# Xinjie-Q/Boosting-NeRV

Hardware: AMD Instinct MI355X
Metric: train frames/sec (higher is better)
Workload: dtype fp32; 1 GPU; NeRV-boost 1.5M (1489577 params, fc_dim 30) train step on a synthetic Bunny-shaped clip 132x3x720x1280: decoder fwd + Fusion10_freq + bwd + fused Adan; frames resident in HBM; global_batch=1, per_gpu_batch=1, parallelism=dp1, hipgraph=True, rccl_ranks=0, collective_in_graph=False

## Files before the change

boosting_nerv_amd/csrc/conv.hip:

```cpp
#include "common.h"
#include "sidejob.h"
#include "conv_common.h"

int bnerv_convbf_try(hipStream_t st, const bnerv_conv_desc& d, int vec, int ksplit, int chunks_per_split);
namespace bnerv_conv { struct KArgs; }
int bnerv_conv4_try(hipStream_t st, bnerv_conv::KArgs& ka);
int bnerv_convs_try(hipStream_t st, const bnerv_conv_desc& d, int vec, int ksplit);
int bnerv_head3_try(hipStream_t st, const bnerv_conv_desc& d);
bool bnerv_convs_shape_ok(const bnerv_conv_desc& d, int vec);
int bnerv_stem_dgrad_try(hipStream_t st, const bnerv_conv_desc& d);
size_t bnerv_stem_dgrad_ws_bytes(const bnerv_conv_desc& d);
int bnerv_convs_tiles(int H, int W);

namespace {
using namespace bnerv_conv;

#ifndef BNERV_ABL
#define BNERV_ABL 0
#endif
constexpr bool ABL_NO_MFMA = BNERV_ABL == 1 || BNERV_ABL == 3 || BNERV_ABL == 4;
constexpr bool ABL_NO_LOAD = BNERV_ABL == 2 || BNERV_ABL == 4;
constexpr bool ABL_NO_STORE = BNERV_ABL == 2 || BNERV_ABL == 3;
struct Item { int g, b, ty0, tx0, tile, ks; };

__device__ __forceinline__ Item decode_item(const KArgs& ka, int it) {
    const int tiles = ka.tiles_x * ka.tiles_y;
    Item r;
    r.ks = 0;
    if (ka.ksplit > 1) { r.ks = it % ka.ksplit; it /= ka.ksplit; }
    r.tile = it % tiles;
    const int rest = it / tiles;
    r.b = rest % ka.d.B;
    r.g = rest / ka.d.B;
    r.ty0 = (r.tile / ka.tiles_x) * TH;
    r.tx0 = (r.tile % ka.tiles_x) * TW;
    return r;
}

template <int IN>
__device__ __forceinline__ float load_in_scalar(const bnerv_conv_desc& d, int b, int ci, int gy, int gx) {
    if constexpr (IN == BNERV_IN_UNSHUFFLE) {
        const int s = d.in_s, s2 = s * s;
        const int c = ci / s2, rem = ci - c * s2, i = rem / s, j = rem - i * s;
        return d.x[(((size_t)b * (d.Cin / s2) + c) * (size_t)(d.H * s) + (size_t)(gy * s + i)) * (size_t)(d.W * s) + (size_t)(gx * s + j)];
    } else {
        const size_t idx = (((size_t)b * d.Cin + ci) * d.H + gy) * (size_t)d.W + gx;
        float sc = 1.f, sh = 0.f, aux = 0.f;
        if constexpr (IN == BNERV_IN_AFFINE || IN == BNERV_IN_GELU_AFFINE) { sc = 1.0f + d.scale[b * d.Cin + ci]; sh = d.shift[b * d.Cin + ci]; }
        if constexpr (IN == BNERV_IN_TANHGRAD) aux = d.aux0[idx];
        return xform1<IN>(d.x[idx], sc, sh, aux);
    }
}

template <int KS, int IN>
__device__ __forceinline__ void stage_scalar(const bnerv_conv_desc& d, float* s_in, int b, int c0, int nch, int ty0, int tx0) {
    using G = Geo<KS>;
    const int n_el = nch * G::PLANE_RAW;
    for (int i0 = threadIdx.x; i0 < n_el; i0 += 256 * 8) {
        float v[8];
// ... 1549 lines not shown
    else BNERV_REQUIRE(d.Cout == d.wCo && d.Cin == d.wCi, "conv_igemm: weight dims mismatch");
    if (d.in_mode == BNERV_IN_AFFINE || d.in_mode == BNERV_IN_GELU_AFFINE) BNERV_REQUIRE(d.scale && d.shift, "conv_igemm: affine prologue needs scale/shift");
    if (d.in_mode == BNERV_IN_TANHGRAD) BNERV_REQUIRE(d.aux0, "conv_igemm: tanh-grad prologue needs aux0");
    if (d.ep_mode == BNERV_EP_BIAS_RES) BNERV_REQUIRE(d.aux0, "conv_igemm: residual epilogue needs aux0");
    if (d.ep_mode == BNERV_EP_DGELU) BNERV_REQUIRE(d.aux0 && d.scale && d.partial && d.out_s == 1, "conv_igemm: DGELU epilogue args");
    if (d.ep_mode == BNERV_EP_DSIN) BNERV_REQUIRE(d.aux0 && d.aux1 && d.scale && d.partial && d.out_s == 1, "conv_igemm: DSIN epilogue args");
    if (d.ep_mode == BNERV_EP_DGELU_SAVED) BNERV_REQUIRE(d.aux0 && d.aux1 && d.scale && d.partial && d.out_s == 1, "conv_igemm: DGELU_SAVED epilogue args");
    if (d.ep_mode == BNERV_EP_BIAS_GELU) BNERV_REQUIRE(d.out_s == 1, "conv_igemm: BIAS_GELU epilogue needs a stride-1 output");
    if (d.in_mode == BNERV_IN_UNSHUFFLE && d.in_s == 1) d.in_mode = BNERV_IN_PLAIN;
    ka.tiles_x = cdiv(d.W, TW);
    ka.tiles_y = cdiv(d.H, TH);
    ka.vec = conv_vec_ok(d);
    hipStream_t st = reinterpret_cast<hipStream_t>(stream);
    ka.ksplit = 1;
    ka.chunks_per_split = 0;
    ka.magic_tiles = ka.magic_tiles_x = 0;
    if (d.ep_mode == BNERV_EP_PLAIN && d.partial != nullptr) {
        const SplitPlan p = plan_split(d);
        ka.ksplit = p.ksplit;
        ka.chunks_per_split = p.chunks_per_split;
    }
    {
        const char* hf = getenv("BNERV_HEAD_FWD");
        if (!(hf && hf[0] == '0') && d.k == 1 && d.in_mode == BNERV_IN_PLAIN && d.ep_mode == BNERV_EP_BIAS_TANH && d.out_s == 1 && ka.vec && !d.transposed &&
            d.Cin == 12 && d.Cout == 3 && d.wCo == 3 && d.wCi == 12 && ((size_t)d.H * d.W) % 4 == 0 && d.B <= 65535) {
            const int hw4 = (int)(((size_t)d.H * d.W) / 4);
            hipLaunchKernelGGL((head1x1_fwd_kernel<3, 12>), dim3(cdiv(hw4, 256), d.B), dim3(256), 0, st, d, hw4);
            BNERV_LAUNCH_CHECK("head1x1_fwd");
            return BNERV_OK;
        }
    }
    if (d.k == 1 && d.in_mode == BNERV_IN_TANHGRAD && d.ep_mode == BNERV_EP_PLAIN && d.out_s == 1 && ka.vec && ka.ksplit == 1 &&
        d.Cin <= HEAD_KMAX && d.Cout <= HEAD_CMAX && ((size_t)d.H * d.W) % 4 == 0 && d.B <= 65535) {
        const int hw4 = (int)(((size_t)d.H * d.W) / 4);
        hipLaunchKernelGGL(head1x1_dgrad_kernel, dim3(cdiv(hw4, 256), d.B), dim3(256), 0, st, d, hw4);
        BNERV_LAUNCH_CHECK("head1x1_dgrad");
        return BNERV_OK;
    }
    if (d.k == 3 && (d.Cout == 3 || d.Cin == 3) && ka.ksplit == 1) {
        const int rh = bnerv_head3_try(st, d);
        if (rh != 1) return rh;
    }
    if (d.ep_mode == BNERV_EP_PLAIN && d.partial != nullptr) {
        const int rs = bnerv_stem_dgrad_try(st, d);
        if (rs != 1) return rs;
    }
    {
        const int rs = bnerv_convs_try(st, d, ka.vec, ka.ksplit);
        if (rs != 1) return rs;
    }
    int rc = bnerv_convbf_try(st, d, ka.vec, ka.ksplit, ka.chunks_per_split);
    if (rc == 1) {
        ka.magic_tiles = ka.magic_tiles_x = 0;
        rc = bnerv_conv4_try(st, ka);
        if (rc == 1) rc = d.k == 1 ? launch_mode<1>(st, ka) : launch_mode<3>(st, ka);
    }
    if (rc != BNERV_OK || ka.ksplit == 1) return rc;
    return bnerv_reduce_slabs(stream, d.partial, ka.ksplit, d.B * d.Cout * d.H * d.W, d.out);
}
```

boosting_nerv_amd/csrc/conv4.hip:

```cpp
#include "conv4_body.h"

namespace {
using namespace bnerv_conv;
using namespace bnerv_q4;

template <int IN, int EP>
__global__ __launch_bounds__(256, 3) void conv_q4_kernel(const KArgs ka, const SidePack side) {
    conv_q4_body<IN, EP>(ka, side, (int)blockIdx.x, (int)gridDim.x);
}

template <int IN, int EP>
int launch_q4(hipStream_t st, KArgs& ka) {
    q4_prepare(ka);
    const size_t lds = q4_lds_bytes();
    static int blocks_per_cu = 0;
    if (blocks_per_cu == 0) {
        int nb = 0;
        if (hipOccupancyMaxActiveBlocksPerMultiprocessor(&nb, reinterpret_cast<const void*>(&conv_q4_kernel<IN, EP>), 256, lds) != hipSuccess || nb < 1) nb = 1;
        blocks_per_cu = nb;
    }
    int grid = 256 * blocks_per_cu;
    if (grid > ka.total_items) grid = ka.total_items;
    SidePack side;
    bnerv_side_take(ka.d.ctx, &side, 2 * grid);
    hipLaunchKernelGGL((conv_q4_kernel<IN, EP>), dim3(grid), dim3(256), lds, st, ka, side);
    BNERV_LAUNCH_CHECK("conv_q4");
    return BNERV_OK;
}

}

#ifdef BNERV_TRACE
extern "C" int bnerv_debug_trace4_read(void* host) { return (int)hipMemcpyFromSymbol(host, HIP_SYMBOL(g_trace4), sizeof(g_trace4)); }
#endif
int bnerv_conv4_try(hipStream_t st, bnerv_conv::KArgs& ka) {
    const bnerv_conv_desc& d = ka.d;
    static const bool off = [] { const char* e = getenv("BNERV_Q4"); return e && e[0] == '0'; }();
    if (off) return 1;
    if (!q4_shape_ok(ka)) return 1;
    const int in = d.in_mode, ep = d.ep_mode;
#define BNERV_CASE(I, E) if (in == I && ep == E) return launch_q4<I, E>(st, ka);
    BNERV_CASE(BNERV_IN_PLAIN, BNERV_EP_BIAS)
    BNERV_CASE(BNERV_IN_PLAIN, BNERV_EP_BIAS_SIN)
    BNERV_CASE(BNERV_IN_PLAIN, BNERV_EP_PLAIN)
    BNERV_CASE(BNERV_IN_PLAIN, BNERV_EP_DGELU_SAVED)
    BNERV_CASE(BNERV_IN_PLAIN, BNERV_EP_DSIN)
#undef BNERV_CASE
    return 1;
}
```

boosting_nerv_amd/csrc/conv4_body.h:

```cpp
#pragma once
#include "common.h"
#include "sidejob.h"
#include "conv_common.h"

namespace bnerv_q4 {
using bnerv_conv::TH; using bnerv_conv::TW; using bnerv_conv::Geo; using bnerv_conv::KArgs; using bnerv_conv::LItem; using bnerv_conv::OOB;
using bnerv_conv::i32x4; using bnerv_conv::make_rsrc; using bnerv_conv::bload; using bnerv_conv::bstore; using bnerv_conv::fast_div;
using bnerv_conv::div_magic; using bnerv_conv::xform1; using bnerv_conv::LEAN_MAX_BYTES;


#ifndef BNERV_ABL4
#define BNERV_ABL4 0
#endif
constexpr int Q4_NCH = 12;
constexpr int Q4_NG = 3;
constexpr int Q4_NQD = 9 * Q4_NG;
constexpr int Q4_NWR = (Q4_NQD + 3) / 4;
constexpr int Q4_QPAD = Q4_NWR * 4;

#ifdef BNERV_TRACE
__device__ unsigned long long g_trace4[1024 * 4 * 6 * 8];
#define TRACE(slot) do { if (lane == 0 && vb < 1024 && trace_iter < 6) g_trace4[((vb * 4 + wave) * 6 + trace_iter) * 8 + (slot)] = __builtin_amdgcn_s_memtime(); } while (0)
#else
#define TRACE(slot) do {} while (0)
#endif

template <int G>
__device__ __forceinline__ f32x4 mfma_q(float a, float w, f32x4 c) {
    return __builtin_amdgcn_mfma_f32_4x4x1f32(a, w, c, 0, 0, 4 + G);
}
__device__ __forceinline__ f32x4 mfma_qsel(int g, float a, float w, f32x4 c) {
    switch (g) {
        case 0: return mfma_q<0>(a, w, c);
        case 1: return mfma_q<1>(a, w, c);
        case 2: return mfma_q<2>(a, w, c);
        default: return mfma_q<3>(a, w, c);
    }
}

__device__ __forceinline__ void dma16(i32x4 rsrc, unsigned voff, unsigned soff, unsigned lds_addr) {
    asm volatile("s_mov_b32 m0, %3\n\tbuffer_load_dwordx4 %0, %1, %2 offen lds" ::"v"(voff), "s"(rsrc), "s"(soff), "s"(lds_addr) : "memory", "m0");
}
template <int N>
__device__ __forceinline__ void q4_wait_dma() {
    asm volatile("s_waitcnt vmcnt(%0)" ::"n"(N) : "memory");
}

template <int IN, int EP>
__device__ __forceinline__ void conv_q4_body(const KArgs& ka, const SidePack& side, const int vb, const int vgrid) {
    using G = Geo<3>;
    constexpr int NSLOT = Q4_NCH * G::ROWS * G::SEGS;
    constexpr int NPRE = (NSLOT + 255) / 256;
    constexpr int S_IN = NPRE * 256 * 4;
    constexpr int S_W = Q4_NCH * Q4_QPAD * 4;
    constexpr bool AFF = (IN == BNERV_IN_AFFINE);
    constexpr bool RED = (EP == BNERV_EP_DSIN || EP == BNERV_EP_DGELU_SAVED);
    constexpr bool TWO_OUT = (EP == BNERV_EP_BIAS_SIN || EP == BNERV_EP_BIAS_GELU);
    static_assert(IN == BNERV_IN_PLAIN || IN == BNERV_IN_AFFINE, "prologues of the 12-channel layers");
    static_assert(G::PLANE == G::PLANE_RAW && S_IN >= Q4_NCH * G::PLANE, "slot offset = 16 * slot index");
    const bnerv_conv_desc& d = ka.d;
    extern __shared__ __attribute__((aligned(16))) float smem[];
    float* s_in = smem;
    float* s_w = smem + 2 * S_IN;
    float* s_red = s_w + S_W;
    float* s_aff = s_red + 256;
    float* s_beta = s_aff + 32;

    const int tid = threadIdx.x, lane = tid & 63;
    const int wave = __builtin_amdgcn_readfirstlane(tid >> 6);
    const int lj = lane & 3, lb = lane >> 2;
    const int Cin = d.Cin, Cout = d.Cout, H = d.H, W = d.W;
    const int tiles_x = ka.tiles_x, tiles_y = ka.tiles_y;
    { const int trace_iter = 5; (void)trace_iter; TRACE(0); }

    const int xcd = vb & 7, lbk = vb >> 3;
    const int nlb = (vgrid - xcd + 7) >> 3;
    const int per = ka.total_items >> 3, extra = ka.total_items & 7;
    const int r0 = xcd * per + min(xcd, extra), r1 = r0 + per + (xcd < extra ? 1 : 0);
    int itx = r0 + lbk;
    if (itx >= r1) { side_run_hosted(side, smem, vb, vgrid); return; }
    const int step_q = fast_div(nlb, ka.magic_tiles_x), step_r = nlb - step_q * tiles_x;
    LItem it;
    {
        const int tiles = tiles_x * tiles_y;
        it.b = fast_div(itx, ka.magic_tiles);
        const int t = itx - it.b * tiles;
        it.ty = fast_div(t, ka.magic_tiles_x);
        it.tx = t - it.ty * tiles_x;
    }
    auto advance = [&](LItem a) {
        a.tx += step_r;
        a.ty += step_q;
        if (a.tx >= tiles_x) { a.tx -= tiles_x; ++a.ty; }
        while (a.ty >= tiles_y) { a.ty -= tiles_y; ++a.b; }
        return a;
    };

    auto slot_geom = [&](int k, int& c, int& r, int& sg) {
        const int sidx = tid + k * 256;
        c = sidx / (G::ROWS * G::SEGS);
        const int rem = sidx - c * (G::ROWS * G::SEGS);
        r = rem / G::SEGS;
        sg = rem - r * G::SEGS;
    };
    auto slot_inside = [&](int k, int ty0, int tx0) {
        int c, r, sg;
        slot_geom(k, c, r, sg);
        const int gy = ty0 + r - G::PAD, gx = tx0 + 4 * sg - G::XOFF;
        return (unsigned)gy < (unsigned)H && (unsigned)gx < (unsigned)W;
    };
    unsigned voff[NPRE];
#pragma unroll
    for (int k = 0; k < NPRE; ++k) {
        int c, r, sg;
        slot_geom(k, c, r, sg);
        voff[k] = (tid + k * 256 < NSLOT && c < Cin) ? (unsigned)(((c * H + r) * W + 4 * sg) * 4) : OOB;
    }
    const unsigned shift = (unsigned)((G::PAD * W + G::XOFF) * 4);
    const unsigned in_bytes = (unsigned)((size_t)d.B * Cin * H * W * 4) + shift;
    const unsigned out_bytes = (unsigned)((size_t)d.B * Cout * H * W * 4);
    i32x4 rx;
    {
        const uintptr_t base = reinterpret_cast<uintptr_t>(d.x) - shift;
        rx[0] = (int)(unsigned)(base & 0xffffffffu);
        rx[1] = (int)(unsigned)((base >> 32) & 0xffffu);
        rx[2] = (int)in_bytes;
        rx[3] = 0x00020000;
    }
    const __amdgpu_buffer_rsrc_t ro = make_rsrc(d.out, 0, out_bytes);
    const __amdgpu_buffer_rsrc_t ro2 = make_rsrc((TWO_OUT && d.out2) ? d.out2 : d.out, 0, out_bytes);
    const __amdgpu_buffer_rsrc_t ra0 = make_rsrc(d.aux0 ? d.aux0 : d.out, 0, out_bytes);
    const __amdgpu_buffer_rsrc_t ra1 = make_rsrc(d.aux1 ? d.aux1 : d.out, 0, out_bytes);
    const __amdgpu_buffer_rsrc_t ra2 = make_rsrc(d.aux2 ? d.aux2 : d.out, 0, out_bytes);
    const unsigned lds_in = (unsigned)(uintptr_t)(__attribute__((address_space(3))) float*)s_in + (unsigned)wave * 1024u;

    const unsigned ovoff = (unsigned)(((lj * H + (lb >> 3)) * W + 4 * (lb & 7)) * 4);
    const unsigned nstep = (unsigned)(4 * H * W * 4);
    float bias_l[Q4_NG];
#pragma unroll
    for (int n = 0; n < Q4_NG; ++n) bias_l[n] = (EP != BNERV_EP_PLAIN && !RED && d.bias && 4 * n + lj < Cout) ? d.bias[4 * n + lj] : 0.f;
    float scl[Q4_NG];
#pragma unroll
    for (int n = 0; n < Q4_NG; ++n) scl[n] = 0.f;

    auto issue = [&](const LItem& a, int buf) {
        const int ty0 = a.ty * TH, tx0 = a.tx * TW;
        const unsigned sb = (unsigned)((((a.b * Cin) * H + ty0) * W + tx0) * 4);
        const unsigned lbase = lds_in + (unsigned)buf * (unsigned)(S_IN * 4);
        const bool interior = ty0 >= G::PAD && ty0 + TH + G::PAD <= H && tx0 >= G::XOFF && tx0 + TW + G::XOFF <= W;
        if (interior) {
#pragma unroll
            for (int k = 0; k < NPRE; ++k) dma16(rx, (BNERV_ABL4 == 2 && d.B > 0) ? OOB : voff[k], sb, lbase + (unsigned)k * 4096u);
        } else {
#pragma unroll
            for (int k = 0; k < NPRE; ++k) dma16(rx, slot_inside(k, ty0, tx0) ? voff[k] : OOB, sb, lbase + (unsigned)k * 4096u);
        }
    };
    auto flush_partials = [&](const LItem& a, const int set) {
        if (wave == 0 && lane < 32) {
            const int q = lane >> 4, c = lane & 15;
            const float* sr = s_red + set * 128;
            const float s = ((sr[(0 * 2 + q) * 16 + c] + sr[(1 * 2 + q) * 16 + c]) + sr[(2 * 2 + q) * 16 + c]) + sr[(3 * 2 + q) * 16 + c];
            const size_t row = (size_t)(a.ty * tiles_x + a.tx) * d.B + a.b;
            if (c < Cout) d.partial[(row * 2 + q) * Cout + c] = s;
        }
    };

    float wr[Q4_NCH][Q4_NWR];
    float beta_l[Q4_NG];
#pragma unroll
    for (int n = 0; n < Q4_NG; ++n) beta_l[n] = 0.f;
    auto fetch_affine = [&](int b) {
        const int c = tid & 15;
        float v = 0.f;
        if (tid < 32 && c < Cin) v = tid < 16 ? 1.0f + d.scale[b * Cin + c] : d.shift[b * Cin + c];
        return v;
    };
    auto load_weights = [&]() {
#pragma unroll
        for (int ci = 0; ci < Q4_NCH; ++ci) {
            const float f = AFF ? s_aff[ci] : 1.0f;
#pragma unroll
            for (int v = 0; v < Q4_NWR; ++v) {
                const float w = s_w[(ci * Q4_QPAD + 4 * v + (lane >> 4)) * 4 + lj];
                wr[ci][v] = AFF ? w * f : w;
            }
        }
    };
    auto fold_shift = [&]() {
        if constexpr (AFF) {
            if (tid < 9 * 16) {
                const int tap = tid >> 4, co = tid & 15;
                float acc_ = 0.f;
                if (co < 4 * Q4_NG) {
#pragma unroll
                    for (int ci = 0; ci < Q4_NCH; ++ci) acc_ = fmaf(s_aff[16 + ci], s_w[(ci * Q4_QPAD + tap * Q4_NG + (co >> 2)) * 4 + (co & 3)], acc_);
                }
                s_beta[tid] = acc_;
            }
            lds_barrier();
#pragma unroll
            for (int n = 0; n < Q4_NG; ++n) {
                float t = 0.f;
#pragma unroll
                for (int tap = 0; tap < 9; ++tap) t += s_beta[tap * 16 + 4 * n + lj];
                beta_l[n] = t;
            }
        }
    };

    int aff_b = -1, ep_b = -1;
    float aff_v = 0.f;
    { const int trace_iter = 5; (void)trace_iter; TRACE(2); }
    if constexpr (AFF) { aff_v = fetch_affine(it.b); aff_b = it.b; }
    issue(it, 0);
    { const int trace_iter = 5; (void)trace_iter; TRACE(3); }
    {
        constexpr int NWV = (S_W + 255) / 256;
        float wv[NWV];
#pragma unroll
        for (int u = 0; u < NWV; ++u) {
            const int e = tid + u * 256;
            const int j = e & 3, cq = e >> 2;
            const int ci = cq / Q4_QPAD, q = cq - ci * Q4_QPAD;
            const int tap = q / Q4_NG, n = q - tap * Q4_NG;
            const int co = 4 * n + j;
            float v = 0.f;
            if (e < S_W && q < Q4_NQD && co < Cout && ci < Cin)
                v = d.transposed ? d.w[(ci * d.wCi + co) * 9 + (8 - tap)] : d.w[(co * d.wCi + ci) * 9 + tap];
            wv[u] = v;
        }
        { const int trace_iter = 5; (void)trace_iter; TRACE(4); }
        if constexpr (AFF) { if (tid < 32) s_aff[tid] = aff_v; }
#pragma unroll
        for (int u = 0; u < NWV; ++u)
            if (tid + u * 256 < S_W) s_w[tid + u * 256] = wv[u];
    }
    q4_wait_dma<0>();
    lds_barrier();
    { const int trace_iter = 5; (void)trace_iter; TRACE(5); }
    load_weights();
    fold_shift();
    { const int trace_iter = 5; (void)trace_iter; TRACE(6); }
    { const int trace_iter = 5; (void)trace_iter; TRACE(1); }
    const float* a_base = s_in + (2 * wave + (lane >> 5)) * G::RS + (lane & 31) + G::COL0;
    int buf = 0;
    LItem prev = it;
    bool have_prev = false;
    int red_set = 0;
    int trace_iter = 0; (void)trace_iter;
    for (; itx < r1; itx += nlb, ++trace_iter, red_set ^= 1) {
        TRACE(0);
        f32x4 acc[Q4_NG];
#pragma unroll
        for (int n = 0; n < Q4_NG; ++n) acc[n] = f32x4{0.f, 0.f, 0.f, 0.f};
        const bool has_next = itx + nlb < r1;
        LItem nxt = it;
        if (has_next) nxt = advance(it);
        TRACE(1);
        if (has_next) issue(nxt, buf ^ 1);
        TRACE(2);
        if constexpr (RED) { if (have_prev) flush_partials(prev, red_set ^ 1); }
        constexpr int NAUX = (EP == BNERV_EP_BIAS_RES) ? 1 : (EP == BNERV_EP_DGELU_SAVED) ? 2 : (EP == BNERV_EP_DSIN) ? 3 : 0;
        f32x4 ax0[NAUX ? Q4_NG : 1], ax1[NAUX >= 2 ? Q4_NG : 1], ax2[NAUX >= 3 ? Q4_NG : 1];
        unsigned so[Q4_NG], vo[Q4_NG];
        bool ch_ok[Q4_NG];
        {
            const int ty0 = it.ty * TH, tx0 = it.tx * TW;
            const unsigned ob = (unsigned)((((it.b * Cout) * H + ty0 + 2 * wave) * W + tx0) * 4);
            const bool full = ty0 + TH <= H && tx0 + TW <= W;
            bool px_ok = true;
            if (!full) px_ok = (ty0 + 2 * wave + (lb >> 3) < H) && (tx0 + 4 * (lb & 7) < W);
#pragma unroll
            for (int n = 0; n < Q4_NG; ++n) {
                so[n] = ob + (unsigned)n * nstep;
                ch_ok[n] = px_ok && (4 * n + lj < Cout);
                vo[n] = (ch_ok[n] && !(BNERV_ABL4 == 2 && d.B > 0)) ? ovoff : OOB;
            }
            if constexpr (NAUX >= 1) {
#pragma unroll
                for (int n = 0; n < Q4_NG; ++n) ax0[n] = bload(ra0, vo[n], so[n]);
            }
            if constexpr (NAUX >= 2) {
#pragma unroll
                for (int n = 0; n < Q4_NG; ++n) ax1[n] = bload(ra1, vo[n], so[n]);
            }
            if constexpr (NAUX >= 3) {
#pragma unroll
                for (int n = 0; n < Q4_NG; ++n) ax2[n] = d.aux2 ? bload(ra2, vo[n], so[n]) : f32x4{1.f, 1.f, 1.f, 1.f};
            }
        }
        float a_cur[3], a_nxt[3];
        if (BNERV_ABL4 != 1 || d.B < 0) {
#pragma unroll
        for (int kx = 0; kx < 3; ++kx) a_cur[kx] = a_base[kx];
#pragma unroll
        for (int ci = 0; ci < Q4_NCH; ++ci) {
#pragma unroll
            for (int ky = 0; ky < 3; ++ky) {
                const int nci = ky == 2 ? ci + 1 : ci, nky = ky == 2 ? 0 : ky + 1;
                if (nci < Q4_NCH) {
#pragma unroll
                    for (int kx = 0; kx < 3; ++kx) a_nxt[kx] = a_base[nci * G::PLANE + nky * G::RS + kx];
                }
                __builtin_amdgcn_sched_barrier(0);
#pragma unroll
                for (int kx = 0; kx < 3; ++kx)
#pragma unroll
                    for (int n = 0; n < Q4_NG; ++n) {
                        const int q = (ky * 3 + kx) * Q4_NG + n;
                        acc[n] = mfma_qsel(q & 3, a_cur[kx], wr[ci][q >> 2], acc[n]);
                    }
                __builtin_amdgcn_sched_barrier(0);
#pragma unroll
                for (int kx = 0; kx < 3; ++kx) a_cur[kx] = a_nxt[kx];
            }
        }
        }
        TRACE(3);
        TRACE(4);
        TRACE(5);
        {
            const int ty0 = it.ty * TH, tx0 = it.tx * TW;
            if constexpr (RED) {
                if (it.b != ep_b) {
#pragma unroll
                    for (int n = 0; n < Q4_NG; ++n) scl[n] = 4 * n + lj < Cout ? 1.0f + d.scale[it.b * Cout + 4 * n + lj] : 0.f;
                    ep_b = it.b;
                }
            }
            if constexpr (RED) {
#pragma unroll
                for (int n = 0; n < Q4_NG; ++n) { if (!ch_ok[n]) acc[n] = f32x4{0.f, 0.f, 0.f, 0.f}; }
            }
            if constexpr (AFF) {
                const bool border = ty0 == 0 || ty0 + TH >= H || tx0 == 0 || tx0 + TW >= W;
                if (!border) {
#pragma unroll
                    for (int n = 0; n < Q4_NG; ++n) acc[n] += beta_l[n];
                } else {
                    const int gy = ty0 + 2 * wave + (lb >> 3), gx0 = tx0 + 4 * (lb & 7);
#pragma unroll
                    for (int n = 0; n < Q4_NG; ++n) {
                        float col[3];
#pragma unroll
                        for (int kx = 0; kx < 3; ++kx) {
                            float t = 0.f;
#pragma unroll
                            for (int ky = 0; ky < 3; ++ky) t += ((unsigned)(gy + ky - 1) < (unsigned)H) ? s_beta[(ky * 3 + kx) * 16 + 4 * n + lj] : 0.f;
                            col[kx] = t;
                        }
#pragma unroll
                        for (int e = 0; e < 4; ++e) {
                            float t = 0.f;
#pragma unroll
                            for (int kx = 0; kx < 3; ++kx) t += ((unsigned)(gx0 + e + kx - 1) < (unsigned)W) ? col[kx] : 0.f;
                            acc[n][e] += t;
                        }
                    }
                }
            }
            if constexpr (EP == BNERV_EP_BIAS || EP == BNERV_EP_PLAIN) {
#pragma unroll
                for (int n = 0; n < Q4_NG; ++n) bstore(ro, vo[n], so[n], acc[n] + bias_l[n]);
            } else if constexpr (EP == BNERV_EP_BIAS_SIN) {
#pragma unroll
                for (int n = 0; n < Q4_NG; ++n) {
                    f32x4 sv, cv;
                    sincos4_f(acc[n] + bias_l[n], &sv, &cv);
                    bstore(ro, vo[n], so[n], sv);
                    bstore(ro2, d.out2 ? vo[n] : OOB, so[n], cv);
                }
            } else if constexpr (EP == BNERV_EP_BIAS_GELU) {
#pragma unroll
                for (int n = 0; n < Q4_NG; ++n) {
                    f32x4 hv, gv;
                    gelu_pair4_f(acc[n] + bias_l[n], &hv, &gv);
                    bstore(ro, vo[n], so[n], hv);
                    bstore(ro2, d.out2 ? vo[n] : OOB, so[n], gv);
                }
            } else if constexpr (EP == BNERV_EP_BIAS_RES) {
#pragma unroll
                for (int n = 0; n < Q4_NG; ++n) bstore(ro, vo[n], so[n], acc[n] + bias_l[n] + ax0[n]);
            } else {
                float ps[Q4_NG], pt[Q4_NG];
#pragma unroll
                for (int n = 0; n < Q4_NG; ++n) {
                    f32x4 r;
                    const f32x4 v = acc[n];
                    ps[n] = 0.f; pt[n] = 0.f;
                    if constexpr (EP == BNERV_EP_DGELU_SAVED) {
#pragma unroll
                        for (int e = 0; e < 4; ++e) { r[e] = v[e] * scl[n] * ax0[n][e]; ps[n] = fmaf(v[e], ax1[n][e], ps[n]); pt[n] += v[e]; }
                    } else {
#pragma unroll
                        for (int e = 0; e < 4; ++e) { r[e] = (ax1[n][e] + v[e] * scl[n]) * ax2[n][e]; ps[n] = fmaf(v[e], ax0[n][e], ps[n]); pt[n] += v[e]; }
                    }
                    bstore(ro, vo[n], so[n], r);
                }
#pragma unroll
                for (int n = 0; n < Q4_NG; ++n) {
#pragma unroll
                    for (int off = 4; off < 64; off <<= 1) {
                        ps[n] += __shfl_xor(ps[n], off, 64);
                        pt[n] += __shfl_xor(pt[n], off, 64);
                    }
                }
                if (lane < 4) {
#pragma unroll
                    for (int n = 0; n < Q4_NG; ++n) { s_red[red_set * 128 + (wave * 2 + 0) * 16 + 4 * n + lane] = ps[n]; s_red[red_set * 128 + (wave * 2 + 1) * 16 + 4 * n + lane] = pt[n]; }
                }
            }
        }
        TRACE(6);
        if (has_next) {
            q4_wait_dma<(TWO_OUT ? 2 : 1) * Q4_NG>();
            lds_barrier();
            if constexpr (AFF) {
                if (nxt.b != aff_b) {
                    const float v = fetch_affine(nxt.b);
                    if (tid < 32) s_aff[tid] = v;
                    lds_barrier();
                    load_weights();
                    fold_shift();
                    aff_b = nxt.b;
                }
            }
            buf ^= 1;
            a_base = s_in + buf * S_IN + (2 * wave + (lane >> 5)) * G::RS + (lane & 31) + G::COL0;
        }
        TRACE(7);
        prev = it;
        have_prev = true;
        it = nxt;
    }
    if constexpr (RED) {
        lds_barrier();
        flush_partials(prev, red_set ^ 1);
    }
    side_run_hosted(side, smem, vb, vgrid);
}


inline size_t q4_lds_bytes() {
    using G = Geo<3>;
    constexpr int NSLOT = Q4_NCH * G::ROWS * G::SEGS;
    constexpr int NPRE = (NSLOT + 255) / 256;
    return ((size_t)2 * NPRE * 256 * 4 + (size_t)Q4_NCH * Q4_QPAD * 4 + 256 + 32 + 9 * 16) * sizeof(float);
}
inline bool q4_shape_ok(const KArgs& ka) {
    const bnerv_conv_desc& d = ka.d;
    const size_t cmax = (size_t)(d.Cin > d.Cout ? d.Cin : d.Cout);
    return ka.vec && d.k == 3 && d.out_s == 1 && d.Cin > 8 && d.Cin <= Q4_NCH && d.Cout <= 4 * Q4_NG && ka.ksplit == 1 &&
           (size_t)d.B * cmax * d.H * d.W * 4 + (size_t)(d.W + 4) * 4 < LEAN_MAX_BYTES;
}
inline void q4_prepare(KArgs& ka) {
    ka.ngroups = 1;
    ka.total_items = ka.d.B * ka.tiles_x * ka.tiles_y;
    ka.nq_total = 3;
    ka.w_resident = 1;
    ka.magic_tiles = div_magic(ka.tiles_x * ka.tiles_y);
    ka.magic_tiles_x = div_magic(ka.tiles_x);
}

}
```

Before: 687.8 frames/s.

## Add Winograd F(2x2,3x3) forward conv kernel for 12-channel full-resolution layers

Adds a Winograd-domain 3x3 convolution kernel that transforms input tiles and filters, multiplies them with fp32 MFMA, and inverse-transforms the result. It is used by default only for the affine-input, bias+residual forward layer at 720x1280 with at most 12 channels, and is gated by the BNERV_WINO environment variable. The affine shift is folded into a per-output beta term, with border correction at image edges. The goal is to cut MFMA and LDS work for these small-channel, high-resolution convolutions, at the cost of extra transform arithmetic and slight numerical differences.

New measurement: 687.3 frames/s (median of 2 runs). About the same (-0.1%).

```diff
diff --git a/boosting_nerv_amd/csrc/conv.hip b/boosting_nerv_amd/csrc/conv.hip
--- a/boosting_nerv_amd/csrc/conv.hip
+++ b/boosting_nerv_amd/csrc/conv.hip
@@ -5,6 +5,7 @@
 int bnerv_convbf_try(hipStream_t st, const bnerv_conv_desc& d, int vec, int ksplit, int chunks_per_split);
 namespace bnerv_conv { struct KArgs; }
 int bnerv_conv4_try(hipStream_t st, bnerv_conv::KArgs& ka);
+int bnerv_convw_try(hipStream_t st, bnerv_conv::KArgs& ka);
 int bnerv_convs_try(hipStream_t st, const bnerv_conv_desc& d, int vec, int ksplit);
 int bnerv_head3_try(hipStream_t st, const bnerv_conv_desc& d);
 bool bnerv_convs_shape_ok(const bnerv_conv_desc& d, int vec);
@@ -1660,7 +1661,8 @@
     int rc = bnerv_convbf_try(st, d, ka.vec, ka.ksplit, ka.chunks_per_split);
     if (rc == 1) {
         ka.magic_tiles = ka.magic_tiles_x = 0;
-        rc = bnerv_conv4_try(st, ka);
+        rc = bnerv_convw_try(st, ka);
+        if (rc == 1) rc = bnerv_conv4_try(st, ka);
         if (rc == 1) rc = d.k == 1 ? launch_mode<1>(st, ka) : launch_mode<3>(st, ka);
     }
     if (rc != BNERV_OK || ka.ksplit == 1) return rc;
diff --git a/boosting_nerv_amd/csrc/convw.hip b/boosting_nerv_amd/csrc/convw.hip
--- /dev/null
+++ b/boosting_nerv_amd/csrc/convw.hip
@@ -0,0 +1,384 @@
+#include "common.h"
+#include "sidejob.h"
+#include "conv_common.h"
+#include <cstdlib>
+
+namespace {
+using namespace bnerv_conv;
+
+constexpr int WN_NCH = 12;
+constexpr int WN_NQ = 3;
+constexpr int WN_SU = WN_NQ * 4 * 64 * 4;
+
+__device__ __forceinline__ void wn_dma16(i32x4 rsrc, unsigned voff, unsigned soff, unsigned lds_addr) {
+    asm volatile("s_mov_b32 m0, %3\n\tbuffer_load_dwordx4 %0, %1, %2 offen lds" ::"v"(voff), "s"(rsrc), "s"(soff), "s"(lds_addr) : "memory", "m0");
+}
+template <int N>
+__device__ __forceinline__ void wn_wait_vm() {
+    asm volatile("s_waitcnt vmcnt(%0)" ::"n"(N) : "memory");
+}
+
+template <int IN, int EP>
+__global__ __launch_bounds__(256, 3) void conv_wino_kernel(const KArgs ka, const SidePack side) {
+    using G = Geo<3>;
+    constexpr int NSLOT = WN_NCH * G::ROWS * G::SEGS;
+    constexpr int NPRE = (NSLOT + 255) / 256;
+    constexpr int S_IN = NPRE * 256 * 4;
+    constexpr bool AFF = (IN == BNERV_IN_AFFINE);
+    constexpr bool TWO_OUT = (EP == BNERV_EP_BIAS_SIN || EP == BNERV_EP_BIAS_GELU);
+    static_assert(IN == BNERV_IN_PLAIN || IN == BNERV_IN_AFFINE, "prologues of the 12-channel layers");
+    static_assert(EP == BNERV_EP_BIAS_SIN || EP == BNERV_EP_BIAS_GELU || EP == BNERV_EP_BIAS_RES, "forward epilogues");
+    static_assert(G::PLANE == G::PLANE_RAW && S_IN >= WN_NCH * G::PLANE, "slot offset = 16 * slot index");
+    const bnerv_conv_desc& d = ka.d;
+    extern __shared__ __attribute__((aligned(16))) float smem[];
+    float* s_in = smem;
+    float* s_u = smem + 2 * S_IN;
+    float* s_aff = s_u + WN_SU;
+    float* s_beta = s_aff + 16;
+
+    const int tid = threadIdx.x, lane = tid & 63;
+    const int wave = __builtin_amdgcn_readfirstlane(tid >> 6);
+    const int li = lane & 15, kq = lane >> 4;
+    const int Cin = d.Cin, Cout = d.Cout, H = d.H, W = d.W;
+    const int tiles_x = ka.tiles_x, tiles_y = ka.tiles_y;
+    const int vb = (int)blockIdx.x, vgrid = (int)gridDim.x;
+
+    const int xcd = vb & 7, lbk = vb >> 3;
+    const int nlb = (vgrid - xcd + 7) >> 3;
+    const int per = ka.total_items >> 3, extra = ka.total_items & 7;
+    const int r0 = xcd * per + min(xcd, extra), r1 = r0 + per + (xcd < extra ? 1 : 0);
+    int itx = r0 + lbk;
+    if (itx >= r1) { side_run_hosted(side, smem, vb, vgrid); return; }
+    const int step_q = fast_div(nlb, ka.magic_tiles_x), step_r = nlb - step_q * tiles_x;
+    LItem it;
+    {
+        const int tiles = tiles_x * tiles_y;
+        it.b = fast_div(itx, ka.magic_tiles);
+        const int t = itx - it.b * tiles;
+        it.ty = fast_div(t, ka.magic_tiles_x);
+        it.tx = t - it.ty * tiles_x;
+    }
+    auto advance = [&](LItem a) {
+        a.tx += step_r;
+        a.ty += step_q;
+        if (a.tx >= tiles_x) { a.tx -= tiles_x; ++a.ty; }
+        while (a.ty >= tiles_y) { a.ty -= tiles_y; ++a.b; }
+        return a;
+    };
+
+    auto slot_geom = [&](int k, int& c, int& r, int& sg) {
+        const int sidx = tid + k * 256;
+        c = sidx / (G::ROWS * G::SEGS);
+        const int rem = sidx - c * (G::ROWS * G::SEGS);
+        r = rem / G::SEGS;
+        sg = rem - r * G::SEGS;
+    };
+    auto slot_inside = [&](int k, int ty0, int tx0) {
+        int c, r, sg;
+        slot_geom(k, c, r, sg);
+        const int gy = ty0 + r - G::PAD, gx = tx0 + 4 * sg - G::XOFF;
+        return (unsigned)gy < (unsigned)H && (unsigned)gx < (unsigned)W;
+    };
+    unsigned voff[NPRE];
+#pragma unroll
+    for (int k = 0; k < NPRE; ++k) {
+        int c, r, sg;
+        slot_geom(k, c, r, sg);
+        voff[k] = (tid + k * 256 < NSLOT && c < Cin) ? (unsigned)(((c * H + r) * W + 4 * sg) * 4) : OOB;
+    }
+    const unsigned shift = (unsigned)((G::PAD * W + G::XOFF) * 4);
+    const unsigned in_bytes = (unsigned)((size_t)d.B * Cin * H * W * 4) + shift;
+    const unsigned out_bytes = (unsigned)((size_t)d.B * Cout * H * W * 4);
+    i32x4 rx;
+    {
+        const uintptr_t base = reinterpret_cast<uintptr_t>(d.x) - shift;
+        rx[0] = (int)(unsigned)(base & 0xffffffffu);
+        rx[1] = (int)(unsigned)((base >> 32) & 0xffffu);
+        rx[2] = (int)in_bytes;
+        rx[3] = 0x00020000;
+    }
+    const __amdgpu_buffer_rsrc_t ro = make_rsrc(d.out, 0, out_bytes);
+    const __amdgpu_buffer_rsrc_t ro2 = make_rsrc((TWO_OUT && d.out2) ? d.out2 : d.out, 0, out_bytes);
+    const __amdgpu_buffer_rsrc_t ra0 = make_rsrc(d.aux0 ? d.aux0 : d.out, 0, out_bytes);
+    const unsigned lds_in = (unsigned)(uintptr_t)(__attribute__((address_space(3))) float*)s_in + (unsigned)wave * 1024u;
+
+    const int co = li;
+    const bool co_ok = co < Cout;
+    const float bias_l = (co_ok && d.bias) ? d.bias[co] : 0.f;
+    float beta_l = 0.f;
+
+    auto issue = [&](const LItem& a, int buf) {
+        const int ty0 = a.ty * TH, tx0 = a.tx * TW;
+        const unsigned sb = (unsigned)((((a.b * Cin) * H + ty0) * W + tx0) * 4);
+        const unsigned lbase = lds_in + (unsigned)buf * (unsigned)(S_IN * 4);
+        const bool interior = ty0 >= G::PAD && ty0 + TH + G::PAD <= H && tx0 >= G::XOFF && tx0 + TW + G::XOFF <= W;
+        if (interior) {
+#pragma unroll
+            for (int k = 0; k < NPRE; ++k) wn_dma16(rx, voff[k], sb, lbase + (unsigned)k * 4096u);
+        } else {
+#pragma unroll
+            for (int k = 0; k < NPRE; ++k) wn_dma16(rx, slot_inside(k, ty0, tx0) ? voff[k] : OOB, sb, lbase + (unsigned)k * 4096u);
+        }
+    };
+
+    auto wval = [&](int o, int i, int tap) { return d.transposed ? d.w[(i * d.wCi + o) * 9 + (8 - tap)] : d.w[(o * d.wCi + i) * 9 + tap]; };
+    auto build_u = [&](int b) {
+        if (tid < WN_NCH * 16) {
+            const int ci = tid >> 4, o = tid & 15;
+            float g[9];
+            const bool ok = ci < Cin && o < Cout;
+            const float f = (AFF && ok) ? 1.0f + d.scale[b * Cin + ci] : 1.0f;
+            int woff = d.transposed ? (ci * d.wCi + o) * 9 + 8 : (o * d.wCi + ci) * 9;
+            asm volatile("" : "+v"(woff));
+            const float* wp = d.w + woff;
+            const int wst = d.transposed ? -1 : 1;
+#pragma unroll
+            for (int t = 0; t < 9; ++t) g[t] = ok ? (AFF ? wp[t * wst] * f : wp[t * wst]) : 0.f;
+            float gg[4][3];
+#pragma unroll
+            for (int kx = 0; kx < 3; ++kx) {
+                const float g0 = g[kx], g1 = g[3 + kx], g2 = g[6 + kx];
+                gg[0][kx] = g0;
+                gg[1][kx] = 0.5f * ((g0 + g1) + g2);
+                gg[2][kx] = 0.5f * ((g0 - g1) + g2);
+                gg[3][kx] = g2;
+            }
+            const int q = ci >> 2, l = (ci & 3) * 16 + o;
+#pragma unroll
+            for (int i = 0; i < 4; ++i) {
+                const float t0 = gg[i][0], t1 = gg[i][1], t2 = gg[i][2];
+                const f32x4 u = {t0, 0.5f * ((t0 + t1) + t2), 0.5f * ((t0 - t1) + t2), t2};
+                *reinterpret_cast<f32x4*>(s_u + ((q * 4 + i) * 64 + l) * 4) = u;
+            }
+        }
+        if constexpr (AFF) {
+            if (tid >= 64 && tid < 64 + WN_NCH) s_aff[tid - 64] = (tid - 64 < Cin) ? d.shift[b * Cin + (tid - 64)] : 0.f;
+        }
+    };
+    auto fold_shift = [&]() {
+        if constexpr (AFF) {
+            if (tid < 9 * 16) {
+                const int tap = tid >> 4, o = tid & 15;
+                float acc_ = 0.f;
+                if (o < Cout) {
+                    for (int ci = 0; ci < Cin; ++ci) acc_ = fmaf(s_aff[ci], wval(o, ci, tap), acc_);
+                }
+                s_beta[tid] = acc_;
+            }
+            lds_barrier();
+            float t = 0.f;
+#pragma unroll
+            for (int tap = 0; tap < 9; ++tap) t += s_beta[tap * 16 + co];
+            beta_l = t;
+        }
+    };
+
+    int aff_b = -1;
+    issue(it, 0);
+
+    const int a_off = kq * G::PLANE + 2 * wave * G::RS + 2 * li + G::COL0;
+    const float* a_base = s_in + a_off;
+    const f32x4* u_base = reinterpret_cast<const f32x4*>(s_u) + lane;
+    int buf = 0;
+    for (; itx < r1; itx += nlb) {
+        if (AFF ? it.b != aff_b : aff_b < 0) {
+            build_u(it.b);
+            wn_wait_vm<0>();
+            lds_barrier();
+            fold_shift();
+            aff_b = it.b;
+        }
+        const bool has_next = itx + nlb < r1;
+        LItem nxt = it;
+        if (has_next) nxt = advance(it);
+        if (has_next) issue(nxt, buf ^ 1);
+        const int ty0 = it.ty * TH, tx0 = it.tx * TW;
+        const unsigned so = (unsigned)((((it.b * Cout) * H + ty0 + 2 * wave) * W + tx0) * 4);
+        unsigned vo[2][2];
+        {
+            const bool full = ty0 + TH <= H && tx0 + TW <= W;
+#pragma unroll
+            for (int r = 0; r < 2; ++r)
+#pragma unroll
+                for (int h = 0; h < 2; ++h) {
+                    const bool ok = co_ok && (full || (ty0 + 2 * wave + r < H && tx0 + 8 * kq + 4 * h < W));
+                    vo[r][h] = ok ? (unsigned)(((co * H + r) * W + 8 * kq + 4 * h) * 4) : OOB;
+                }
+        }
+
+        f32x4 acc[16];
+#pragma unroll
+        for (int p = 0; p < 16; ++p) acc[p] = f32x4{0.f, 0.f, 0.f, 0.f};
+        float dd[4][4];
+        f32x4 ub[4];
+        auto read_quad = [&](int q) {
+            const float* pb = a_base + q * 4 * G::PLANE;
+#pragma unroll
+            for (int r = 0; r < 4; ++r)
+#pragma unroll
+                for (int c = 0; c < 4; ++c) dd[r][c] = pb[r * G::RS + c];
+#pragma unroll
+            for (int j = 0; j < 4; ++j) ub[j] = u_base[(q * 4 + j) * 64];
+        };
+        read_quad(0);
+#pragma unroll
+        for (int q = 0; q < WN_NQ; ++q) {
+            float t[4][4];
+#pragma unroll
+            for (int c = 0; c < 4; ++c) {
+                t[0][c] = dd[0][c] - dd[2][c];
+                t[1][c] = dd[1][c] + dd[2][c];
+                t[2][c] = dd[2][c] - dd[1][c];
+                t[3][c] = dd[1][c] - dd[3][c];
+            }
+            float v[16];
+#pragma unroll
+            for (int r = 0; r < 4; ++r) {
+                v[4 * r + 0] = t[r][0] - t[r][2];
+                v[4 * r + 1] = t[r][1] + t[r][2];
+                v[4 * r + 2] = t[r][2] - t[r][1];
+                v[4 * r + 3] = t[r][1] - t[r][3];
+            }
+            f32x4 uc[4];
+#pragma unroll
+            for (int j = 0; j < 4; ++j) uc[j] = ub[j];
+            __builtin_amdgcn_sched_barrier(0);
+            if (q + 1 < WN_NQ) read_quad(q + 1);
+#pragma unroll
+            for (int p = 0; p < 16; ++p) acc[p] = __builtin_amdgcn_mfma_f32_16x16x4f32(v[p], uc[p >> 2][p & 3], acc[p], 0, 0, 0);
+            __builtin_amdgcn_sched_barrier(0);
+        }
+
+        f32x4 ax[2][2];
+        if constexpr (EP == BNERV_EP_BIAS_RES) {
+#pragma unroll
+            for (int r = 0; r < 2; ++r)
+#pragma unroll
+                for (int h = 0; h < 2; ++h) ax[r][h] = bload(ra0, vo[r][h], so);
+        }
+        f32x4 y[2][2];
+#pragma unroll
+        for (int i = 0; i < 4; ++i) {
+            float s0[4], s1[4];
+#pragma unroll
+            for (int c = 0; c < 4; ++c) {
+                s0[c] = (acc[c][i] + acc[4 + c][i]) + acc[8 + c][i];
+                s1[c] = (acc[4 + c][i] - acc[8 + c][i]) - acc[12 + c][i];
+            }
+            y[0][i >> 1][2 * (i & 1) + 0] = (s0[0] + s0[1]) + s0[2];
+            y[0][i >> 1][2 * (i & 1) + 1] = (s0[1] - s0[2]) - s0[3];
+            y[1][i >> 1][2 * (i & 1) + 0] = (s1[0] + s1[1]) + s1[2];
+            y[1][i >> 1][2 * (i & 1) + 1] = (s1[1] - s1[2]) - s1[3];
+        }
+        if constexpr (AFF) {
+            const bool border = ty0 == 0 || ty0 + TH >= H || tx0 == 0 || tx0 + TW >= W;
+            if (!border) {
+#pragma unroll
+                for (int r = 0; r < 2; ++r)
+#pragma unroll
+                    for (int h = 0; h < 2; ++h) y[r][h] += beta_l;
+            } else {
+#pragma unroll
+                for (int r = 0; r < 2; ++r) {
+                    const int gy = ty0 + 2 * wave + r;
+                    float col[3];
+#pragma unroll
+                    for (int kx = 0; kx < 3; ++kx) {
+                        float t = 0.f;
+#pragma unroll
+                        for (int ky = 0; ky < 3; ++ky) t += ((unsigned)(gy + ky - 1) < (unsigned)H) ? s_beta[(ky * 3 + kx) * 16 + co] : 0.f;
+                        col[kx] = t;
+                    }
+#pragma unroll
+                    for (int h = 0; h < 2; ++h) {
+                        const int gx0 = tx0 + 8 * kq + 4 * h;
+#pragma unroll
+                        for (int e = 0; e < 4; ++e) {
+                            float t = 0.f;
+#pragma unroll
+                            for (int kx = 0; kx < 3; ++kx) t += ((unsigned)(gx0 + e + kx - 1) < (unsigned)W) ? col[kx] : 0.f;
+                            y[r][h][e] += t;
+                        }
+                    }
+                }
+            }
+        }
+#pragma unroll
+        for (int r = 0; r < 2; ++r)
+#pragma unroll
+            for (int h = 0; h < 2; ++h) {
+                if constexpr (EP == BNERV_EP_BIAS_SIN) {
+                    f32x4 sv, cv;
+                    sincos4_f(y[r][h] + bias_l, &sv, &cv);
+                    bstore(ro, vo[r][h], so, sv);
+                    bstore(ro2, d.out2 ? vo[r][h] : OOB, so, cv);
+                } else if constexpr (EP == BNERV_EP_BIAS_GELU) {
+                    f32x4 hv, gv;
+                    gelu_pair4_f(y[r][h] + bias_l, &hv, &gv);
+                    bstore(ro, vo[r][h], so, hv);
+                    bstore(ro2, d.out2 ? vo[r][h] : OOB, so, gv);
+                } else {
+                    bstore(ro, vo[r][h], so, y[r][h] + bias_l + ax[r][h]);
+                }
+            }
+        if (has_next) {
+            wn_wait_vm<(TWO_OUT ? 2 : 1) * 4>();
+            lds_barrier();
+            buf ^= 1;
+            a_base = s_in + buf * S_IN + a_off;
+        }
+        it = nxt;
+    }
+    side_run_hosted(side, smem, vb, vgrid);
+}
+
+inline size_t wino_lds_bytes() {
+    using G = Geo<3>;
+    constexpr int NSLOT = WN_NCH * G::ROWS * G::SEGS;
+    constexpr int NPRE = (NSLOT + 255) / 256;
+    return ((size_t)2 * NPRE * 256 * 4 + WN_SU + 16 + 9 * 16) * sizeof(float);
+}
+
+template <int IN, int EP>
+int launch_wino(hipStream_t st, KArgs& ka) {
+    ka.ngroups = 1;
+    ka.total_items = ka.d.B * ka.tiles_x * ka.tiles_y;
+    ka.nq_total = 3;
+    ka.w_resident = 1;
+    ka.magic_tiles = div_magic(ka.tiles_x * ka.tiles_y);
+    ka.magic_tiles_x = div_magic(ka.tiles_x);
+    const size_t lds = wino_lds_bytes();
+    static int blocks_per_cu = 0;
+    if (blocks_per_cu == 0) {
+        int nb = 0;
+        if (hipOccupancyMaxActiveBlocksPerMultiprocessor(&nb, reinterpret_cast<const void*>(&conv_wino_kernel<IN, EP>), 256, lds) != hipSuccess || nb < 1) nb = 1;
+        blocks_per_cu = nb;
+    }
+    int grid = 256 * blocks_per_cu;
+    if (grid > ka.total_items) grid = ka.total_items;
+    SidePack side;
+    bnerv_side_take(ka.d.ctx, &side, 2 * grid);
+    hipLaunchKernelGGL((conv_wino_kernel<IN, EP>), dim3(grid), dim3(256), lds, st, ka, side);
+    BNERV_LAUNCH_CHECK("conv_wino");
+    return BNERV_OK;
+}
+
+}
+
+int bnerv_convw_try(hipStream_t st, bnerv_conv::KArgs& ka) {
+    const bnerv_conv_desc& d = ka.d;
+    const char* e = getenv("BNERV_WINO");
+    if (e && e[0] == '0') return 1;
+    const bool all = e && e[0] == '2';
+    const size_t cmax = (size_t)(d.Cin > d.Cout ? d.Cin : d.Cout);
+    if (!(ka.vec && d.k == 3 && d.out_s == 1 && d.Cin > 8 && d.Cin <= WN_NCH && d.Cout <= 12 && ka.ksplit == 1 &&
+          (size_t)d.B * cmax * d.H * d.W * 4 + (size_t)(d.W + 4) * 4 < LEAN_MAX_BYTES))
+        return 1;
+    const int in = d.in_mode, ep = d.ep_mode;
+    if (in == BNERV_IN_AFFINE && ep == BNERV_EP_BIAS_RES && (all || (size_t)d.H * d.W >= (size_t)720 * 1280))
+        return launch_wino<BNERV_IN_AFFINE, BNERV_EP_BIAS_RES>(st, ka);
+    if (!all) return 1;
+    if (in == BNERV_IN_AFFINE && ep == BNERV_EP_BIAS_GELU) return launch_wino<BNERV_IN_AFFINE, BNERV_EP_BIAS_GELU>(st, ka);
+    if (in == BNERV_IN_PLAIN && ep == BNERV_EP_BIAS_SIN) return launch_wino<BNERV_IN_PLAIN, BNERV_EP_BIAS_SIN>(st, ka);
+    return 1;
+}
```

## Enable q4 conv path for affine-prologue layers via in-LDS affine transform

Applied to the files above, without the earlier changes.

Routes the 12-channel affine-input layers (BIAS_GELU and BIAS_RES epilogues) through the q4 MFMA conv kernel. The earlier approach folded scale into the weights and shift into a per-tap beta with a costly border correction. It is replaced by an elementwise affine pass over the staged input tile in LDS after each DMA, masked for out-of-image slots. The MFMA loop order is also remapped for the affine case. Debug launch counters are added as well. This adds an LDS read-modify-write pass per tile and a barrier, and removes the weight reloads on batch change and the epilogue border math.

New measurement: 688.9 frames/s before, 702.9 frames/s after (median of 6 runs). 2.0% higher.

```diff
diff --git a/boosting_nerv_amd/csrc/conv4.hip b/boosting_nerv_amd/csrc/conv4.hip
--- a/boosting_nerv_amd/csrc/conv4.hip
+++ b/boosting_nerv_amd/csrc/conv4.hip
@@ -1,8 +1,12 @@
+#include <atomic>
 #include "conv4_body.h"
 
 namespace {
 using namespace bnerv_conv;
 using namespace bnerv_q4;
+
+std::atomic<long long> g_q4_launches[2];
+std::atomic<int> g_q4_last_grid{0};
 
 template <int IN, int EP>
 __global__ __launch_bounds__(256, 3) void conv_q4_kernel(const KArgs ka, const SidePack side) {
@@ -25,6 +29,8 @@
     bnerv_side_take(ka.d.ctx, &side, 2 * grid);
     hipLaunchKernelGGL((conv_q4_kernel<IN, EP>), dim3(grid), dim3(256), lds, st, ka, side);
     BNERV_LAUNCH_CHECK("conv_q4");
+    g_q4_launches[IN == BNERV_IN_AFFINE ? 1 : 0].fetch_add(1, std::memory_order_relaxed);
+    g_q4_last_grid.store(grid, std::memory_order_relaxed);
     return BNERV_OK;
 }
 
@@ -33,6 +39,10 @@
 #ifdef BNERV_TRACE
 extern "C" int bnerv_debug_trace4_read(void* host) { return (int)hipMemcpyFromSymbol(host, HIP_SYMBOL(g_trace4), sizeof(g_trace4)); }
 #endif
+extern "C" long long bnerv_debug_q4_launches(int affine, int* last_grid) {
+    if (last_grid) *last_grid = g_q4_last_grid.load(std::memory_order_relaxed);
+    return g_q4_launches[affine ? 1 : 0].load(std::memory_order_relaxed);
+}
 int bnerv_conv4_try(hipStream_t st, bnerv_conv::KArgs& ka) {
     const bnerv_conv_desc& d = ka.d;
     static const bool off = [] { const char* e = getenv("BNERV_Q4"); return e && e[0] == '0'; }();
@@ -45,6 +55,8 @@
     BNERV_CASE(BNERV_IN_PLAIN, BNERV_EP_PLAIN)
     BNERV_CASE(BNERV_IN_PLAIN, BNERV_EP_DGELU_SAVED)
     BNERV_CASE(BNERV_IN_PLAIN, BNERV_EP_DSIN)
+    BNERV_CASE(BNERV_IN_AFFINE, BNERV_EP_BIAS_GELU)
+    BNERV_CASE(BNERV_IN_AFFINE, BNERV_EP_BIAS_RES)
 #undef BNERV_CASE
     return 1;
 }
diff --git a/boosting_nerv_amd/csrc/conv4_body.h b/boosting_nerv_amd/csrc/conv4_body.h
--- a/boosting_nerv_amd/csrc/conv4_body.h
+++ b/boosting_nerv_amd/csrc/conv4_body.h
@@ -64,7 +64,6 @@
     float* s_w = smem + 2 * S_IN;
     float* s_red = s_w + S_W;
     float* s_aff = s_red + 256;
-    float* s_beta = s_aff + 32;
 
     const int tid = threadIdx.x, lane = tid & 63;
     const int wave = __builtin_amdgcn_readfirstlane(tid >> 6);
@@ -167,45 +166,45 @@
     };
 
     float wr[Q4_NCH][Q4_NWR];
-    float beta_l[Q4_NG];
-#pragma unroll
-    for (int n = 0; n < Q4_NG; ++n) beta_l[n] = 0.f;
+    auto load_weights = [&]() {
+#pragma unroll
+        for (int ci = 0; ci < Q4_NCH; ++ci)
+#pragma unroll
+            for (int v = 0; v < Q4_NWR; ++v) wr[ci][v] = s_w[(ci * Q4_QPAD + 4 * v + (lane >> 4)) * 4 + lj];
+    };
+    float sc[AFF ? NPRE : 1], sh[AFF ? NPRE : 1];
     auto fetch_affine = [&](int b) {
         const int c = tid & 15;
         float v = 0.f;
         if (tid < 32 && c < Cin) v = tid < 16 ? 1.0f + d.scale[b * Cin + c] : d.shift[b * Cin + c];
         return v;
     };
-    auto load_weights = [&]() {
-#pragma unroll
-        for (int ci = 0; ci < Q4_NCH; ++ci) {
-            const float f = AFF ? s_aff[ci] : 1.0f;
-#pragma unroll
-            for (int v = 0; v < Q4_NWR; ++v) {
-                const float w = s_w[(ci * Q4_QPAD + 4 * v + (lane >> 4)) * 4 + lj];
-                wr[ci][v] = AFF ? w * f : w;
-            }
-        }
-    };
-    auto fold_shift = [&]() {
-        if constexpr (AFF) {
-            if (tid < 9 * 16) {
-                const int tap = tid >> 4, co = tid & 15;
-                float acc_ = 0.f;
-                if (co < 4 * Q4_NG) {
-#pragma unroll
-                    for (int ci = 0; ci < Q4_NCH; ++ci) acc_ = fmaf(s_aff[16 + ci], s_w[(ci * Q4_QPAD + tap * Q4_NG + (co >> 2)) * 4 + (co & 3)], acc_);
-                }
-                s_beta[tid] = acc_;
-            }
-            lds_barrier();
-#pragma unroll
-            for (int n = 0; n < Q4_NG; ++n) {
-                float t = 0.f;
-#pragma unroll
-                for (int tap = 0; tap < 9; ++tap) t += s_beta[tap * 16 + 4 * n + lj];
-                beta_l[n] = t;
-            }
+    auto pick_affine = [&]() {
+#pragma unroll
+        for (int k = 0; k < (AFF ? NPRE : 0); ++k) {
+            int c, r, sg;
+            slot_geom(k, c, r, sg);
+            const bool ok = voff[k] != OOB;
+            sc[k] = ok ? s_aff[c & 15] : 0.f;
+            sh[k] = ok ? s_aff[16 + (c & 15)] : 0.f;
+        }
+    };
+    auto affine_pass = [&](const LItem& a, int buf_) {
+        const int ty0 = a.ty * TH, tx0 = a.tx * TW;
+        const bool interior = ty0 >= G::PAD && ty0 + TH + G::PAD <= H && tx0 >= G::XOFF && tx0 + TW + G::XOFF <= W;
+        float* base = s_in + buf_ * S_IN + 4 * tid;
+#pragma unroll
+        for (int k = 0; k < (AFF ? NPRE : 0); ++k) {
+            float s = sc[k], h = sh[k];
+            if (!interior) {
+                const bool ok = slot_inside(k, ty0, tx0);
+                s = ok ? s : 0.f;
+                h = ok ? h : 0.f;
+            }
+            f32x4 v = *reinterpret_cast<const f32x4*>(base + k * 1024);
+#pragma unroll
+            for (int e = 0; e < 4; ++e) v[e] = xform1<IN>(v[e], s, h, 0.f);
+            *reinterpret_cast<f32x4*>(base + k * 1024) = v;
         }
     };
 
@@ -240,7 +239,11 @@
     lds_barrier();
     { const int trace_iter = 5; (void)trace_iter; TRACE(5); }
     load_weights();
-    fold_shift();
+    if constexpr (AFF) {
+        pick_affine();
+        affine_pass(it, 0);
+        lds_barrier();
+    }
     { const int trace_iter = 5; (void)trace_iter; TRACE(6); }
     { const int trace_iter = 5; (void)trace_iter; TRACE(1); }
     const float* a_base = s_in + (2 * wave + (lane >> 5)) * G::RS + (lane & 31) + G::COL0;
@@ -290,31 +293,34 @@
                 for (int n = 0; n < Q4_NG; ++n) ax2[n] = d.aux2 ? bload(ra2, vo[n], so[n]) : f32x4{1.f, 1.f, 1.f, 1.f};
             }
         }
+        auto kpos = [](int j, int e, int& ci, int& ky, int& kx) {
+            if constexpr (AFF) { const int tap = j >> 2; ci = 3 * (j & 3) + e; ky = tap / 3; kx = tap - 3 * ky; }
+            else { ci = j / 3; ky = j - 3 * ci; kx = e; }
+        };
         float a_cur[3], a_nxt[3];
         if (BNERV_ABL4 != 1 || d.B < 0) {
 #pragma unroll
-        for (int kx = 0; kx < 3; ++kx) a_cur[kx] = a_base[kx];
-#pragma unroll
-        for (int ci = 0; ci < Q4_NCH; ++ci) {
-#pragma unroll
-            for (int ky = 0; ky < 3; ++ky) {
-                const int nci = ky == 2 ? ci + 1 : ci, nky = ky == 2 ? 0 : ky + 1;
-                if (nci < Q4_NCH) {
-#pragma unroll
-                    for (int kx = 0; kx < 3; ++kx) a_nxt[kx] = a_base[nci * G::PLANE + nky * G::RS + kx];
-                }
-                __builtin_amdgcn_sched_barrier(0);
-#pragma unroll
-                for (int kx = 0; kx < 3; ++kx)
-#pragma unroll
-                    for (int n = 0; n < Q4_NG; ++n) {
-                        const int q = (ky * 3 + kx) * Q4_NG + n;
-                        acc[n] = mfma_qsel(q & 3, a_cur[kx], wr[ci][q >> 2], acc[n]);
-                    }
-                __builtin_amdgcn_sched_barrier(0);
-#pragma unroll
-                for (int kx = 0; kx < 3; ++kx) a_cur[kx] = a_nxt[kx];
-            }
+        for (int e = 0; e < 3; ++e) { int ci, ky, kx; kpos(0, e, ci, ky, kx); a_cur[e] = a_base[ci * G::PLANE + ky * G::RS + kx]; }
+#pragma unroll
+        for (int j = 0; j < 3 * Q4_NCH; ++j) {
+            if (j + 1 < 3 * Q4_NCH) {
+#pragma unroll
+                for (int e = 0; e < 3; ++e) { int ci, ky, kx; kpos(j + 1, e, ci, ky, kx); a_nxt[e] = a_base[ci * G::PLANE + ky * G::RS + kx]; }
+            }
+            __builtin_amdgcn_sched_barrier(0);
+#pragma unroll
+            for (int e = 0; e < 3; ++e) {
+                int ci, ky, kx;
+                kpos(j, e, ci, ky, kx);
+#pragma unroll
+                for (int n = 0; n < Q4_NG; ++n) {
+                    const int q = (ky * 3 + kx) * Q4_NG + n;
+                    acc[n] = mfma_qsel(q & 3, a_cur[e], wr[ci][q >> 2], acc[n]);
+                }
+            }
+            __builtin_amdgcn_sched_barrier(0);
+#pragma unroll
+            for (int e = 0; e < 3; ++e) a_cur[e] = a_nxt[e];
         }
         }
         TRACE(3);
@@ -333,33 +339,6 @@
 #pragma unroll
                 for (int n = 0; n < Q4_NG; ++n) { if (!ch_ok[n]) acc[n] = f32x4{0.f, 0.f, 0.f, 0.f}; }
             }
-            if constexpr (AFF) {
-                const bool border = ty0 == 0 || ty0 + TH >= H || tx0 == 0 || tx0 + TW >= W;
-                if (!border) {
-#pragma unroll
-                    for (int n = 0; n < Q4_NG; ++n) acc[n] += beta_l[n];
-                } else {
-                    const int gy = ty0 + 2 * wave + (lb >> 3), gx0 = tx0 + 4 * (lb & 7);
-#pragma unroll
-                    for (int n = 0; n < Q4_NG; ++n) {
-                        float col[3];
-#pragma unroll
-                        for (int kx = 0; kx < 3; ++kx) {
-                            float t = 0.f;
-#pragma unroll
-                            for (int ky = 0; ky < 3; ++ky) t += ((unsigned)(gy + ky - 1) < (unsigned)H) ? s_beta[(ky * 3 + kx) * 16 + 4 * n + lj] : 0.f;
-                            col[kx] = t;
-                        }
-#pragma unroll
-                        for (int e = 0; e < 4; ++e) {
-                            float t = 0.f;
-#pragma unroll
-                            for (int kx = 0; kx < 3; ++kx) t += ((unsigned)(gx0 + e + kx - 1) < (unsigned)W) ? col[kx] : 0.f;
-                            acc[n][e] += t;
-                        }
-                    }
-                }
-            }
             if constexpr (EP == BNERV_EP_BIAS || EP == BNERV_EP_PLAIN) {
 #pragma unroll
                 for (int n = 0; n < Q4_NG; ++n) bstore(ro, vo[n], so[n], acc[n] + bias_l[n]);
@@ -415,17 +394,17 @@
         TRACE(6);
         if (has_next) {
             q4_wait_dma<(TWO_OUT ? 2 : 1) * Q4_NG>();
-            lds_barrier();
             if constexpr (AFF) {
                 if (nxt.b != aff_b) {
                     const float v = fetch_affine(nxt.b);
                     if (tid < 32) s_aff[tid] = v;
                     lds_barrier();
-                    load_weights();
-                    fold_shift();
+                    pick_affine();
                     aff_b = nxt.b;
                 }
-            }
+                affine_pass(nxt, buf ^ 1);
+            }
+            lds_barrier();
             buf ^= 1;
             a_base = s_in + buf * S_IN + (2 * wave + (lane >> 5)) * G::RS + (lane & 31) + G::COL0;
         }
@@ -446,7 +425,7 @@
     using G = Geo<3>;
     constexpr int NSLOT = Q4_NCH * G::ROWS * G::SEGS;
     constexpr int NPRE = (NSLOT + 255) / 256;
-    return ((size_t)2 * NPRE * 256 * 4 + (size_t)Q4_NCH * Q4_QPAD * 4 + 256 + 32 + 9 * 16) * sizeof(float);
+    return ((size_t)2 * NPRE * 256 * 4 + (size_t)Q4_NCH * Q4_QPAD * 4 + 256 + 32) * sizeof(float);
 }
 inline bool q4_shape_ok(const KArgs& ka) {
     const bnerv_conv_desc& d = ka.d;
```
